# halajun/VDO_SLAM

Hardware: AMD Instinct MI355X
Metric: frames/sec (per-frame hot path, KITTI-0000-shaped 1242x375) + ms/LM-iter (batch factor graph) (higher is better)
Workload: dtype f64 (LM, RANSAC) / u8,i32,f32 (front-end, tracking)

## Files before the change

### vdo_slam_amd/csrc/orb.hip

```cpp
#include <algorithm>
#include <atomic>
#include <chrono>
#include <cmath>
#include <condition_variable>
#include <functional>
#include <memory>
#include <mutex>
#include <thread>
#include <cstring>
#include <vector>

#include "../../include/vdo_slam_hip.h"
#include "ctx.hpp"
#include "host_pool.hpp"
#include "orb_match.hpp"
#include "orb_pattern.hpp"

namespace vdo {

constexpr int kEdge = 19, kHalfPatch = 15, kPatch = 31;
constexpr int kSpecCand = 24576;
constexpr int kMaxCellDim = 68;
static_assert(kMaxCellDim <= 128, "k_fast_cells packs cell-local coordinates in 7 bits");

// ... 532 lines not shown
      int best = idx[n.b];
      float mr = resp[best];
      for (int k = n.b + 1; k < n.e; ++k) if (resp[idx[k]] > mr) { best = idx[k]; mr = resp[best]; }
      out.push_back(best);
    }
  }

 private:
  const float *x = nullptr, *y = nullptr, *resp = nullptr;
  std::vector<int> idx, tmp, ini_cnt, ini_fill;
  std::vector<int> cls;
  std::vector<QNode> nodes;
  std::vector<std::pair<int, int>> sizeAndNode, prevSN;
  int head = -1, tail = -1, count = 0;
  int push_back(const QNode& n) {
    nodes.push_back(n);
    const int id = (int)nodes.size() - 1;
    nodes[id].prev = tail; nodes[id].next = -1;
    if (tail != -1) nodes[tail].next = id; else head = id;
    tail = id; ++count;
    return id;
  }
  int push_front(const QNode& n) {
    nodes.push_back(n);
    const int id = (int)nodes.size() - 1;
    nodes[id].prev = -1; nodes[id].next = head;
    if (head != -1) nodes[head].prev = id; else tail = id;
    head = id; ++count;
    return id;
  }
  void erase(int id) {
    const QNode n = nodes[id];
    if (n.prev != -1) nodes[n.prev].next = n.next; else head = n.next;
    if (n.next != -1) nodes[n.next].prev = n.prev; else tail = n.prev;
    --count;
  }
  void divide_and_add(int id, int* nToExpand) {
    QNode c[4];
    const QNode n = nodes[id];
    const int halfX = (int)std::ceil((float)(n.URx - n.ULx) / 2), halfY = (int)std::ceil((float)(n.BRy - n.ULy) / 2);
    QNode &n1 = c[0], &n2 = c[1], &n3 = c[2], &n4 = c[3];
    n1.ULx = n.ULx; n1.ULy = n.ULy; n1.URx = n.ULx + halfX; n1.URy = n.ULy; n1.BLx = n.ULx; n1.BLy = n.ULy + halfY; n1.BRx = n.ULx + halfX; n1.BRy = n.ULy + halfY;
    n2.ULx = n1.URx; n2.ULy = n1.URy; n2.URx = n.URx; n2.URy = n.URy; n2.BLx = n1.BRx; n2.BLy = n1.BRy; n2.BRx = n.URx; n2.BRy = n.ULy + halfY;
    n3.ULx = n1.BLx; n3.ULy = n1.BLy; n3.URx = n1.BRx; n3.URy = n1.BRy; n3.BLx = n.BLx; n3.BLy = n.BLy; n3.BRx = n1.BRx; n3.BRy = n.BLy;
    n4.ULx = n3.URx; n4.ULy = n3.URy; n4.URx = n2.BRx; n4.URy = n2.BRy; n4.BLx = n3.BRx; n4.BLy = n3.BRy; n4.BRx = n.BRx; n4.BRy = n.BRy;
    int cnt[4] = {0, 0, 0, 0};
    const float sx = (float)n1.URx, sy = (float)n1.BRy;
    for (int k = n.b; k < n.e; ++k) {
      const int ki = idx[k];
      const int q = (x[ki] < sx) ? ((y[ki] < sy) ? 0 : 2) : ((y[ki] < sy) ? 1 : 3);
      cls[k] = q; ++cnt[q];
    }
    int cur[4];
    cur[0] = n.b; cur[1] = cur[0] + cnt[0]; cur[2] = cur[1] + cnt[1]; cur[3] = cur[2] + cnt[2];
    for (int q = 0; q < 4; ++q) { c[q].b = cur[q]; c[q].e = cur[q] + cnt[q]; c[q].noMore = cnt[q] == 1; }
    for (int k = n.b; k < n.e; ++k) tmp[cur[cls[k]]++] = idx[k];
    std::memcpy(idx.data() + n.b, tmp.data() + n.b, sizeof(int) * (size_t)(n.e - n.b));
    for (int q = 0; q < 4; ++q) {
      if (cnt[q] == 0) continue;
      const int nid = push_front(c[q]);
      if (cnt[q] > 1) {
        if (nToExpand) ++*nToExpand;
        sizeAndNode.push_back(std::make_pair(cnt[q], nid));
      }
    }
  }
};

constexpr int kQtThreads = 1024, kQtMaxNodes = 1024, kQtLdsKeys = 4096, kQtMaxCand = 32768, kQtMaxRounds = 48;
enum { kQtOk = 0, kQtHostLevel = 1, kQtCandOverflow = 2, kQtNodeOverflow = 3, kQtRoundCap = 4, kQtBadStrip = 5 };
struct QtDesc {
  int on_device;
  int N, nIni, H;
  int node_cap;
  int cand_cap;
  int koff;
  int out_off;
  float hX;
  float scale;
  int pad[2];
};
typedef unsigned long long qt_u64;

__device__ __forceinline__ int qt_field(qt_u64 v, int q) { return (int)((v >> (16 * q)) & 0xffffu); }
__device__ __forceinline__ int qt_nchild(qt_u64 v) { return (qt_field(v, 0) != 0) + (qt_field(v, 1) != 0) + (qt_field(v, 2) != 0) + (qt_field(v, 3) != 0); }
__device__ __forceinline__ int qt_nexp(qt_u64 v) { return (qt_field(v, 0) > 1) + (qt_field(v, 1) > 1) + (qt_field(v, 2) > 1) + (qt_field(v, 3) > 1); }

__device__ __forceinline__ qt_u64 qt_block_scan(qt_u64 v, qt_u64* s_w, qt_u64& total) {
  const int lane = threadIdx.x & 63, wv = threadIdx.x >> 6;
  qt_u64 inc = v;
#pragma unroll
  for (int off = 1; off < 64; off <<= 1) { const qt_u64 u = __shfl_up(inc, off, 64); if (lane >= off) inc += u; }
  __syncthreads();
  if (lane == 63) s_w[wv] = inc;
  __syncthreads();
  qt_u64 base = 0, tot = 0;
#pragma unroll
  for (int w = 0; w < kQtThreads / 64; ++w) { const qt_u64 p = s_w[w]; if (w < wv) base += p; tot += p; }
  total = tot;
  return base + inc - v;
}

__global__ __launch_bounds__(kQtThreads) void k_quadtree(const QtDesc* __restrict__ qd, const int* __restrict__ level_cnt,
                                                         const float* __restrict__ ox, const float* __restrict__ oy, const float* __restrict__ oresp,
                                                         uint32_t* wi, qt_u64* wp, int* __restrict__ dsel, int* __restrict__ dhdr,
                                                         int* __restrict__ hsel, int* __restrict__ hhdr) {
  __shared__ uint32_t s_nx[2][kQtMaxNodes], s_ny[2][kQtMaxNodes];
  __shared__ int s_b[2][kQtMaxNodes], s_e[2][kQtMaxNodes], s_cid[2][kQtMaxNodes];
  __shared__ qt_u64 s_qc[kQtMaxNodes];
  __shared__ qt_u64 s_sc[kQtMaxNodes];
  __shared__ int s_rank[kQtMaxNodes], s_order[kQtMaxNodes], s_nb[kQtMaxNodes];
  __shared__ qt_u64 s_w[kQtThreads / 64];
  __shared__ int s_m;
  __shared__ uint32_t s_xy[kQtLdsKeys];
  __shared__ uint16_t s_idx[2][kQtLdsKeys], s_kn[2][kQtLdsKeys];
  __shared__ qt_u64 s_P[kQtLdsKeys + 1];
  __shared__ uint8_t s_resp[kQtLdsKeys];
  const int l = blockIdx.x, t = threadIdx.x;
  const QtDesc D = qd[l];
  auto finish = [&](int status, int count) { if (t == 0) { dhdr[l] = hhdr[l] = count; dhdr[16 + l] = hhdr[16 + l] = status; } };
  if (!D.on_device) { finish(kQtHostLevel, 0); return; }
  int pos = 0;
  for (int q = 0; q < l; ++q) pos += level_cnt[q];
  const int n = level_cnt[l];
  if (n > D.cand_cap) { finish(kQtCandOverflow, 0); return; }
  if (n <= 0) { finish(kQtOk, 0); return; }
  const float *x = ox + pos, *y = oy + pos, *resp = oresp + pos;
  const int KC = (n + kQtThreads - 1) / kQtThreads;
  const int k0 = min(t * KC, n), k1 = min(k0 + KC, n);
  const int N = D.N, cap = D.node_cap;

  const bool lds_keys = n <= kQtLdsKeys;
  auto run = [&](uint32_t* xy, uint16_t* idA, uint16_t* idB, uint16_t* knA, uint16_t* knB, qt_u64* P) __attribute__((always_inline)) {
    {
      int bad = 0;
      for (int k = k0; k < k1; ++k) {
        const float fx = x[k], fy = y[k];
        const int s = (int)__fdiv_rn(fx, D.hX);
        bad |= (s < 0 || s >= D.nIni || !(fx >= 0.f && fx < 65536.f && fy >= 0.f && fy < 65536.f));
        xy[k] = (uint32_t)(int)fx | ((uint32_t)(int)fy << 16);
        if (lds_keys) { const float r = resp[k]; bad |= !(r >= 0.f && r < 256.f); s_resp[k] = (uint8_t)(int)r; }
      }
      if (__syncthreads_or(bad)) { finish(kQtBadStrip, 0); return; }
      int base = 0;
      for (int g = 0; g < D.nIni; g += 4) {
        qt_u64 a = 0;
        for (int k = k0; k < k1; ++k) { const int s = (int)__fdiv_rn((float)(xy[k] & 0xffffu), D.hX) - g; if (s >= 0 && s < 4) a += 1ull << (16 * s); }
        qt_u64 tot;
        qt_u64 ex = qt_block_scan(a, s_w, tot);
        int st[5];
        st[0] = base;
        for (int j = 0; j < 4; ++j) st[j + 1] = st[j] + qt_field(tot, j);
        for (int k = k0; k < k1; ++k) {
          const int s = (int)__fdiv_rn((float)(xy[k] & 0xffffu), D.hX) - g;
          if (s < 0 || s >= 4) continue;
          const int p = st[s] + qt_field(ex, s);
          if ((unsigned)p < (unsigned)n) { idA[p] = (uint16_t)k; knA[p] = (uint16_t)(g + s); }
          ex += 1ull << (16 * s);
        }
        if (t < 4 && g + t < D.nIni) {
          const int i = g + t;
          const int sx0 = (int)(D.hX * (float)i), sx1 = (int)(D.hX * (float)(i + 1));
          s_nx[1][i] = (uint32_t)sx0 | ((uint32_t)sx1 << 16); s_ny[1][i] = (uint32_t)D.H << 16;
          s_b[1][i] = st[t]; s_e[1][i] = st[t + 1];
        }
        base = st[4];
      }
      __syncthreads();
    }
    int count;
    {
      const int NC = (D.nIni + kQtThreads - 1) / kQtThreads;
      const int i0 = min(t * NC, D.nIni), i1 = min(i0 + NC, D.nIni);
      int a = 0;
      for (int i = i0; i < i1; ++i) a += s_e[1][i] > s_b[1][i];
      qt_u64 tot;
      int ex = (int)qt_block_scan((qt_u64)a, s_w, tot);
      count = (int)tot;
      for (int i = i0; i < i1; ++i) {
        s_nb[i] = ex;
        if (s_e[1][i] > s_b[1][i]) { s_nx[0][ex] = s_nx[1][i]; s_ny[0][ex] = s_ny[1][i]; s_b[0][ex] = s_b[1][i]; s_e[0][ex] = s_e[1][i]; s_cid[0][ex] = i; ++ex; }
      }
      __syncthreads();
      for (int k = k0; k < k1; ++k) knA[k] = (uint16_t)s_nb[knA[k]];
      __syncthreads();
    }
    int c = 0, next_cid = D.nIni;
    bool final_phase = false;
    for (int round = 0;; ++round) {
      if (round >= kQtMaxRounds) { finish(kQtRoundCap, 0); return; }
      const int o = c ^ 1;
      const uint16_t *idc = c ? idB : idA, *knc = c ? knB : knA;
      uint16_t *ido = c ? idA : idB, *kno = c ? knA : knB;
      {
        auto quadrant = [&](int k) {
          const int i = knc[k];
          if (s_e[c][i] - s_b[c][i] <= 1) return 4;
          const uint32_t nx = s_nx[c][i], ny = s_ny[c][i];
          const int x0 = (int)(nx & 0xffffu), x1 = (int)(nx >> 16), y0 = (int)(ny & 0xffffu), y1 = (int)(ny >> 16);
          const int mx = x0 + ((x1 - x0 + 1) >> 1), my = y0 + ((y1 - y0 + 1) >> 1);
          const uint32_t v = xy[idc[k]];
          const int kx = (int)(v & 0xffffu), ky = (int)(v >> 16);
          return (kx < mx) ? ((ky < my) ? 0 : 2) : ((ky < my) ? 1 : 3);
        };
        qt_u64 a = 0;
        uint32_t qs = 0;
        for (int k = k0; k < k1; ++k) { const int q = quadrant(k); if (q < 4) a += 1ull << (16 * q); if (k - k0 < 8) qs |= (uint32_t)q << (4 * (k - k0)); }
        qt_u64 tot;
        qt_u64 ex = qt_block_scan(a, s_w, tot);
        for (int k = k0; k < k1; ++k) { P[k] = ex; const int q = k - k0 < 8 ? (int)((qs >> (4 * (k - k0))) & 15u) : quadrant(k); if (q < 4) ex += 1ull << (16 * q); }
        if (t == 0) P[n] = tot;
        __syncthreads();
      }
      const int NC = (count + kQtThreads - 1) / kQtThreads;
      const int i0 = min(t * NC, count), i1 = min(i0 + NC, count);
      int E;
      {
        int a = 0;
        for (int i = i0; i < i1; ++i) {
          const int b = s_b[c][i], e = s_e[c][i];
          const bool ex = e - b > 1;
          s_qc[i] = ex ? P[e] - P[b] : 0ull;
          a += ex;
        }
        qt_u64 tot;
        int r = (int)qt_block_scan((qt_u64)a, s_w, tot);
        E = (int)tot;
        if (!final_phase) {
          for (int i = i0; i < i1; ++i) {
            if (s_e[c][i] - s_b[c][i] <= 1) { s_rank[i] = -1; continue; }
            s_rank[i] = r; s_order[r] = i; ++r;
          }
        } else {
          for (int i = i0; i < i1; ++i) {
            const int sz = s_e[c][i] - s_b[c][i];
            s_sc[i] = sz > 1 ? ((qt_u64)sz << 32) | (uint32_t)s_cid[c][i] : 0ull;
            s_rank[i] = sz > 1 ? 0 : -1;
          }
          __syncthreads();
          const int G = max(1, kQtThreads / count), per = kQtThreads / G, part = t % G;
          for (int i = t / G; i < count; i += per) {
            const qt_u64 ki = s_sc[i];
            if (!ki) continue;
            int rk = 0;
#pragma unroll 4
            for (int j = part; j < count; j += G) rk += s_sc[j] > ki;
            if (rk) atomicAdd(&s_rank[i], rk);
          }
          __syncthreads();
          for (int i = i0; i < i1; ++i) if (s_rank[i] >= 0) s_order[s_rank[i]] = i;
        }
        if (t == 0) s_m = E;
        __syncthreads();
      }
      {
        const int RC = (E + kQtThreads - 1) / kQtThreads;
        const int r0 = min(t * RC, E), r1 = min(r0 + RC, E);
        qt_u64 a = 0;
        for (int r = r0; r < r1; ++r) { const qt_u64 qc = s_qc[s_order[r]]; a += (qt_u64)qt_nchild(qc) | ((qt_u64)qt_nexp(qc) << 32); }
        qt_u64 tot;
        qt_u64 ex = qt_block_scan(a, s_w, tot);
        for (int r = r0; r < r1; ++r) {
          const qt_u64 qc = s_qc[s_order[r]];
          ex += (qt_u64)qt_nchild(qc) | ((qt_u64)qt_nexp(qc) << 32);
          s_sc[r] = ex;
          if (final_phase && count + (int)(ex & 0xffffffffu) - (r + 1) >= N) atomicMin(&s_m, r + 1);
        }
        __syncthreads();
      }
      const int m = s_m;
      const int TC = m > 0 ? (int)(s_sc[m - 1] & 0xffffffffu) : 0, n_to_expand = m > 0 ? (int)(s_sc[m - 1] >> 32) : 0;
      const int new_count = TC + count - m;
      if (new_count > cap) { finish(kQtNodeOverflow, 0); return; }
      {
        int a = 0;
        for (int i = i0; i < i1; ++i) { const int rk = s_rank[i]; a += !(rk >= 0 && rk < m); }
        qt_u64 tot;
        int u = (int)qt_block_scan((qt_u64)a, s_w, tot);
        for (int i = i0; i < i1; ++i) {
          const int rk = s_rank[i];
          if (!(rk >= 0 && rk < m)) {
            const int p = TC + u++;
            s_nx[o][p] = s_nx[c][i]; s_ny[o][p] = s_ny[c][i]; s_b[o][p] = s_b[c][i]; s_e[o][p] = s_e[c][i]; s_cid[o][p] = s_cid[c][i];
            s_nb[i] = p;
            continue;
          }
          const qt_u64 qc = s_qc[i];
          const int incl = (int)(s_sc[rk] & 0xffffffffu), nch = qt_nchild(qc);
          const int nbase = TC - incl;
          s_nb[i] = nbase;
          const uint32_t nx = s_nx[c][i], ny = s_ny[c][i];
          const int x0 = (int)(nx & 0xffffu), x1 = (int)(nx >> 16), y0 = (int)(ny & 0xffffu), y1 = (int)(ny >> 16);
          const int mx = x0 + ((x1 - x0 + 1) >> 1), my = y0 + ((y1 - y0 + 1) >> 1);
          int b = s_b[c][i], made = 0;
          for (int q = 0; q < 4; ++q) {
            const int sz = qt_field(qc, q);
            if (!sz) continue;
            const int p = nbase + nch - 1 - made;
            s_nx[o][p] = (q & 1) ? ((uint32_t)mx | ((uint32_t)x1 << 16)) : ((uint32_t)x0 | ((uint32_t)mx << 16));
            s_ny[o][p] = (q & 2) ? ((uint32_t)my | ((uint32_t)y1 << 16)) : ((uint32_t)y0 | ((uint32_t)my << 16));
            s_b[o][p] = b; s_e[o][p] = b + sz; s_cid[o][p] = next_cid + incl - nch + made;
            b += sz; ++made;
          }
        }
        __syncthreads();
      }
      for (int k = k0; k < k1; ++k) {
        const int i = knc[k], rk = s_rank[i];
        int nk = k, nn = s_nb[i];
        if (rk >= 0 && rk < m) {
          const qt_u64 qc = s_qc[i], pk = P[k], d = P[k + 1] - pk;
          const int q = (d & 0xffffu) ? 0 : ((d >> 16) & 0xffffu) ? 1 : ((d >> 32) & 0xffffu) ? 2 : 3;
          const int b = s_b[c][i];
          int offq = 0, after = 0;
          for (int j = 0; j < 4; ++j) { const int sz = qt_field(qc, j); if (j < q) offq += sz; else if (j > q) after += sz != 0; }
          nk = b + offq + qt_field(pk, q) - qt_field(P[b], q);
          nn += after;
        }
        if ((unsigned)nk < (unsigned)n) { ido[nk] = idc[k]; kno[nk] = (uint16_t)nn; }
      }
      __syncthreads();
      c = o; next_cid += TC;
      const int prev = count;
      count = new_count;
      if (count >= N || count == prev) break;
      if (!final_phase && count + 3 * n_to_expand > N) final_phase = true;
    }
    const uint16_t* idc = c ? idB : idA;
    for (int i = t; i < count; i += kQtThreads) {
      const int b = s_b[c][i], e = s_e[c][i];
      int best = idc[b];
      if (lds_keys) {
        int mr = s_resp[best];
        for (int k = b + 1; k < e; ++k) { const int ki = idc[k], r = s_resp[ki]; if (r > mr) { best = ki; mr = r; } }
      } else {
        float mr = resp[best];
        for (int k = b + 1; k < e; ++k) { const int ki = idc[k]; const float r = resp[ki]; if (r > mr) { best = ki; mr = r; } }
      }
      hsel[D.out_off + i] = best; dsel[D.out_off + i] = pos + best;
    }
    finish(kQtOk, count);
  };
  if (n <= kQtLdsKeys) run(s_xy, s_idx[0], s_idx[1], s_kn[0], s_kn[1], s_P);
  else {
    uint32_t* const w0 = wi + 3 * (size_t)D.koff;
    uint16_t* const h0 = (uint16_t*)(w0 + D.cand_cap);
    run(w0, h0, h0 + D.cand_cap, h0 + 2 * (size_t)D.cand_cap, h0 + 3 * (size_t)D.cand_cap, wp + D.koff + l);
  }
}

__global__ __launch_bounds__(256) void k_qt_rows(const QtDesc* __restrict__ qd, int n_levels, const int* __restrict__ dhdr, const int* __restrict__ dsel,
                                                 const float* __restrict__ ox, const float* __restrict__ oy, const float* __restrict__ oresp,
                                                 const uint8_t* __restrict__ pyr, const LevelDesc* __restrict__ levels, UMax um, float* __restrict__ hrows, int row_pitch) {
  const int lane = threadIdx.x & 31;
  const int slot = (blockIdx.x * 256 + threadIdx.x) >> 5;
  int l = -1;
  for (int q = 0; q < n_levels; ++q) { const int off = qd[q].out_off; if (qd[q].on_device && slot >= off && slot < off + qd[q].node_cap) l = q; }
  const bool valid = l >= 0 && dhdr[16 + l] == kQtOk && slot - qd[l].out_off < dhdr[l];
  int m10 = 0, m01 = 0, kx = 0, ky = 0, dense = 0;
  if (valid) {
    dense = dsel[slot];
    kx = (int)ox[dense]; ky = (int)oy[dense];
    if (lane < 31) {
      const LevelDesc L = levels[l];
      const int v = lane - kHalfPatch;
      const int d = um.v[v < 0 ? -v : v];
      const uint8_t* row = pyr + L.off_inner + (size_t)(ky + (kEdge - 3) + v) * L.bw + (kx + (kEdge - 3));
      int px[kPatch];
#pragma unroll
      for (int u = 0; u < kPatch; ++u) px[u] = row[u - kHalfPatch];
      int rs = 0;
#pragma unroll
      for (int u = 0; u < kPatch; ++u) { const int uu = u - kHalfPatch; const int p = (uu >= -d && uu <= d) ? px[u] : 0; m10 += uu * p; rs += p; }
      m01 = v * rs;
    }
  }
#pragma unroll
  for (int off = 16; off > 0; off >>= 1) { m10 += __shfl_down(m10, off, 32); m01 += __shfl_down(m01, off, 32); }
  if (valid && lane == 0) {
    const float ang = fast_atan2_dev((float)m01, (float)m10);
    float fx = (float)kx + (float)(kEdge - 3), fy = (float)ky + (float)(kEdge - 3);
    if (l != 0) { const float sc = qd[l].scale; fx = fx * sc; fy = fy * sc; }
    float* r = hrows + slot;
    r[0] = fx; r[row_pitch] = fy; r[2 * (size_t)row_pitch] = oresp[dense]; r[3 * (size_t)row_pitch] = ang;
  }
}

}

using namespace vdo;

struct vdo_orb {
  vdo_ctx* ctx = nullptr;
  vdo_orb_params prm{};
  int w = 0, h = 0, ncells = 0;
  int max_kp = 0;
  int cell_cap = 1;
  std::vector<LevelDesc> levels;
  std::vector<CellDesc> cells;
  std::vector<int> cell_level, nfeat;
  std::vector<float> scale;
  UMax um{};
  Blur7 blur{};
  PyrDesc pyr{};
  PyrDesc pyr2{};
  std::vector<void*> allocs;
  uint8_t *d_src = nullptr, *d_pyr = nullptr, *d_blur = nullptr;
  LevelDesc* d_levels = nullptr; CellDesc* d_cells = nullptr; int* d_cell_level = nullptr;
  int *d_cnt = nullptr, *d_offs = nullptr, *d_level_cnt = nullptr; uint32_t* d_pack = nullptr;
  float *d_x = nullptr, *d_y = nullptr, *d_resp = nullptr, *d_ang = nullptr; int* d_lvl = nullptr;
  int64_t pyr_bytes = 0, blur_bytes = 0;
  int dense_cap = 0;
  std::vector<int> sel_dense;
  OrbPattern* d_pat = nullptr; int* d_sel = nullptr; uint8_t* d_desc = nullptr; int desc_cap = 0;
  bool desc_ready = false, pos_ready = false;
  float *m_x = nullptr, *m_y = nullptr; int32_t* m_oct = nullptr; int match_cap = 0;
  float* h_pin = nullptr; float* d_pin = nullptr;
  bool fused_angle = false;
  const float *hx = nullptr, *hy = nullptr, *hresp = nullptr, *hang = nullptr; std::vector<int> hlevel_cnt;
  int n_cand = 0;
  QuadTree qt[16];
  std::vector<int> sel[16];
  std::unique_ptr<LevelPool> pool;
  bool dev_tree = false;
  bool ang_queued = false;
  QtDesc qtd[16]; QtDesc* d_qtd = nullptr;
  int qt_out = 0;
  uint32_t* d_qt_i = nullptr; int *d_qsel = nullptr, *d_qhdr = nullptr; qt_u64* d_qt_p = nullptr;
  double ms_device = 0, ms_tree = 0;
  bool begun = false;
// ... 618 lines not shown
  if (n_features) *n_features = o->nfeat[level];
  if (n_candidates) *n_candidates = o->hlevel_cnt.empty() ? 0 : o->hlevel_cnt[level];
  return VDO_OK;
}

extern "C" int vdo_orb_get_pyramid(vdo_orb* o, int level, uint8_t* out_bordered) {
  if (!o || !out_bordered || level < 0 || level >= o->prm.n_levels) return set_error(VDO_ERR_INVALID, "bad argument");
  int rc = ctx_bind(o->ctx);
  if (rc != VDO_OK) return rc;
  const LevelDesc& L = o->levels[level];
  if (hipMemcpy(out_bordered, o->d_pyr + L.off, (size_t)L.bw * L.bh, hipMemcpyDeviceToHost) != hipSuccess) return set_error(VDO_ERR_NO_DEVICE, "D2H failed");
  return VDO_OK;
}

extern "C" int vdo_orb_get_blurred(vdo_orb* o, int level, uint8_t* out) {
  if (!o || !out || level < 0 || level >= o->prm.n_levels) return set_error(VDO_ERR_INVALID, "bad argument");
  int rc = ctx_bind(o->ctx);
  if (rc != VDO_OK) return rc;
  int64_t boff = 0;
  for (int l = 0; l < level; ++l) boff += (int64_t)o->levels[l].w * o->levels[l].h;
  const LevelDesc& L = o->levels[level];
  hipStreamSynchronize(o->ctx->stream);
  if (hipMemcpy(out, o->d_blur + boff, (size_t)L.w * L.h, hipMemcpyDeviceToHost) != hipSuccess) return set_error(VDO_ERR_NO_DEVICE, "D2H failed");
  return VDO_OK;
}

extern "C" int vdo_orb_get_candidates(vdo_orb* o, int level, float* x, float* y, float* resp, float* angle, int cap, int* n) {
  if (!o || !n || level < 0 || level >= o->prm.n_levels || o->hlevel_cnt.empty()) return set_error(VDO_ERR_INVALID, "bad argument / no extraction yet");
  int pos = 0;
  for (int l = 0; l < level; ++l) pos += o->hlevel_cnt[l];
  const int cnt = o->hlevel_cnt[level];
  *n = cnt;
  if (angle && !o->fused_angle && !o->begun) {
    const int rc = ctx_bind(o->ctx);
    if (rc != VDO_OK) return rc;
    orb_ensure_angles(o);
  }
  if (angle && !o->fused_angle && !o->begun && hipEventSynchronize(o->ev_ang) != hipSuccess) return set_error(VDO_ERR_NO_DEVICE, "orb angle stage failed: %s", hipGetErrorString(hipGetLastError()));
  for (int k = 0; k < cnt && k < cap; ++k) {
    if (x) x[k] = o->hx[pos + k];
    if (y) y[k] = o->hy[pos + k];
    if (resp) resp[k] = o->hresp[pos + k];
    if (angle) angle[k] = o->hang[pos + k];
  }
  return VDO_OK;
}

extern "C" int vdo_depth_preprocess(vdo_ctx* ctx, float* depth, int64_t n, float bf, float factor, int is_device) {
  if (!ctx || !depth || n <= 0) return set_error(VDO_ERR_INVALID, "bad argument");
  int rc = ctx_bind(ctx);
  if (rc != VDO_OK) return rc;
  hipStream_t s = ctx->stream;
  float* d = depth;
  if (!is_device) {
    if (hipMalloc((void**)&d, 4 * (size_t)n) != hipSuccess) return set_error(VDO_ERR_OOM, "hipMalloc failed");
    hipMemcpyAsync(d, depth, 4 * (size_t)n, hipMemcpyHostToDevice, s);
  }
  hipLaunchKernelGGL(k_depth_preprocess, dim3((unsigned)((n + 255) / 256)), dim3(256), 0, s, d, n, bf, factor);
  if (!is_device) {
    hipMemcpyAsync(depth, d, 4 * (size_t)n, hipMemcpyDeviceToHost, s);
    hipStreamSynchronize(s);
    hipFree(d);
  }
  hipError_t e = hipGetLastError();
  if (e != hipSuccess) return set_error(VDO_ERR_NO_DEVICE, "depth preprocess: %s", hipGetErrorString(e));
  return VDO_OK;
}

extern "C" int vdo_rgb2gray(vdo_ctx* ctx, const uint8_t* rgb, int64_t n_pixels, int channels, int rgb_order, uint8_t* gray) {
  if (!ctx || !rgb || !gray || n_pixels <= 0 || (channels != 3 && channels != 4)) return set_error(VDO_ERR_INVALID, "bad argument");
  int rc = ctx_bind(ctx);
  if (rc != VDO_OK) return rc;
  hipStream_t s = ctx->stream;
  uint8_t *ds = nullptr, *dd = nullptr;
  if (hipMalloc((void**)&ds, (size_t)n_pixels * channels) != hipSuccess || hipMalloc((void**)&dd, (size_t)n_pixels) != hipSuccess) { if (ds) hipFree(ds); return set_error(VDO_ERR_OOM, "hipMalloc failed"); }
  hipMemcpyAsync(ds, rgb, (size_t)n_pixels * channels, hipMemcpyHostToDevice, s);
  hipLaunchKernelGGL(k_rgb2gray, dim3((unsigned)((n_pixels + 255) / 256)), dim3(256), 0, s, (const uint8_t*)ds, n_pixels, channels, rgb_order, dd);
  hipMemcpyAsync(gray, dd, (size_t)n_pixels, hipMemcpyDeviceToHost, s);
  hipError_t e = hipStreamSynchronize(s);
  hipFree(ds); hipFree(dd);
  if (e != hipSuccess) return set_error(VDO_ERR_NO_DEVICE, "rgb2gray: %s", hipGetErrorString(e));
  return VDO_OK;
}
```

Measured before the change: 1497.

## Restructure quadtree kernel with DPP block scans and one-node-per-thread rounds

Replaces the shuffle-based block prefix scan with DPP row/wave scans and readlane, which removes one barrier per scan and double-buffers the wave-total slots. The per-round node processing now maps one node per thread, fusing the separate count/rank/child scans into a single packed scan. Keys and node ids, and node begin/end, are packed into 32-bit words, and the split points are cached. Candidate loops are batched by four to overlap LDS loads. It also adds an optional compile-time profiling hook. The DPP control codes and the packing assumptions add correctness risk.

```diff
diff --git a/vdo_slam_amd/csrc/orb.hip b/vdo_slam_amd/csrc/orb.hip
--- a/vdo_slam_amd/csrc/orb.hip
+++ b/vdo_slam_amd/csrc/orb.hip
@@ -638,23 +638,59 @@
 };
 typedef unsigned long long qt_u64;
 
-__device__ __forceinline__ int qt_field(qt_u64 v, int q) { return (int)((v >> (16 * q)) & 0xffffu); }
+#ifdef QT_PROFILE
+constexpr int kQtProfCap = 1024;
+__device__ long long g_qt_prof[4 + 2 * kQtProfCap];
+#define QT_STAMP(id)                                                                                      \
+  do {                                                                                                    \
+    if (blockIdx.x == 0 && threadIdx.x == 0 && qt_pn < kQtProfCap) {                                      \
+      if (qt_pn == 0) g_qt_prof[1] = (long long)wall_clock64();                                           \
+      g_qt_prof[4 + 2 * qt_pn] = (id); g_qt_prof[5 + 2 * qt_pn] = (long long)clock64();                   \
+      g_qt_prof[0] = ++qt_pn; g_qt_prof[2] = (long long)wall_clock64();                                   \
+    }                                                                                                     \
+  } while (0)
+#else
+#define QT_STAMP(id) do {} while (0)
+#endif
+
+__device__ __forceinline__ int qt_field(qt_u64 v, int q) { const uint32_t h = (q & 2) ? (uint32_t)(v >> 32) : (uint32_t)v; return (int)((h >> ((q & 1) << 4)) & 0xffffu); }
 __device__ __forceinline__ int qt_nchild(qt_u64 v) { return (qt_field(v, 0) != 0) + (qt_field(v, 1) != 0) + (qt_field(v, 2) != 0) + (qt_field(v, 3) != 0); }
 __device__ __forceinline__ int qt_nexp(qt_u64 v) { return (qt_field(v, 0) > 1) + (qt_field(v, 1) > 1) + (qt_field(v, 2) > 1) + (qt_field(v, 3) > 1); }
 
+static_assert(kQtMaxCand < 65536 && 4 * kQtMaxNodes < 65536, "a field of a packed scan word overflows into its neighbour: the halves can no longer be scanned apart");
+static_assert(kQtThreads / 64 == 16 && kQtMaxNodes <= kQtThreads, "16 wave totals = one DPP row; one node per thread");
+template <int CTRL, int ROWS>
+__device__ __forceinline__ uint32_t qt_dpp(uint32_t v) { return (uint32_t)__builtin_amdgcn_update_dpp(0, (int)v, CTRL, ROWS, 0xF, false); }
+__device__ __forceinline__ uint32_t qt_row_scan(uint32_t v) {
+  v += qt_dpp<0x111, 0xF>(v); v += qt_dpp<0x112, 0xF>(v); v += qt_dpp<0x114, 0xF>(v); v += qt_dpp<0x118, 0xF>(v);
+  return v;
+}
+__device__ __forceinline__ uint32_t qt_wave_scan(uint32_t v) {
+  v = qt_row_scan(v);
+  v += qt_dpp<0x142, 0xA>(v); v += qt_dpp<0x143, 0xC>(v);
+  return v;
+}
 __device__ __forceinline__ qt_u64 qt_block_scan(qt_u64 v, qt_u64* s_w, qt_u64& total) {
-  const int lane = threadIdx.x & 63, wv = threadIdx.x >> 6;
-  qt_u64 inc = v;
-#pragma unroll
-  for (int off = 1; off < 64; off <<= 1) { const qt_u64 u = __shfl_up(inc, off, 64); if (lane >= off) inc += u; }
-  __syncthreads();
+  const int lane = threadIdx.x & 63, wv = __builtin_amdgcn_readfirstlane((int)(threadIdx.x >> 6));
+  const qt_u64 inc = (qt_u64)qt_wave_scan((uint32_t)v) | ((qt_u64)qt_wave_scan((uint32_t)(v >> 32)) << 32);
   if (lane == 63) s_w[wv] = inc;
   __syncthreads();
-  qt_u64 base = 0, tot = 0;
-#pragma unroll
-  for (int w = 0; w < kQtThreads / 64; ++w) { const qt_u64 p = s_w[w]; if (w < wv) base += p; tot += p; }
-  total = tot;
-  return base + inc - v;
+  const qt_u64 p = s_w[lane & 15];
+  const uint32_t lo = qt_row_scan((uint32_t)p), hi = qt_row_scan((uint32_t)(p >> 32));
+  total = (qt_u64)(uint32_t)__builtin_amdgcn_readlane((int)lo, 15) | ((qt_u64)(uint32_t)__builtin_amdgcn_readlane((int)hi, 15) << 32);
+  const int pw = wv > 0 ? wv - 1 : 0;
+  const qt_u64 before = (qt_u64)(uint32_t)__builtin_amdgcn_readlane((int)lo, pw) | ((qt_u64)(uint32_t)__builtin_amdgcn_readlane((int)hi, pw) << 32);
+  return (wv > 0 ? before : 0ull) + inc - v;
+}
+__device__ __forceinline__ int qt_block_scan32(int v, qt_u64* s_w, int& total) {
+  const int lane = threadIdx.x & 63, wv = __builtin_amdgcn_readfirstlane((int)(threadIdx.x >> 6));
+  const uint32_t inc = qt_wave_scan((uint32_t)v);
+  if (lane == 63) s_w[wv] = inc;
+  __syncthreads();
+  const uint32_t lo = qt_row_scan((uint32_t)s_w[lane & 15]);
+  total = __builtin_amdgcn_readlane((int)lo, 15);
+  const int before = __builtin_amdgcn_readlane((int)lo, wv > 0 ? wv - 1 : 0);
+  return (wv > 0 ? before : 0) + (int)inc - v;
 }
 
 __global__ __launch_bounds__(kQtThreads) void k_quadtree(const QtDesc* __restrict__ qd, const int* __restrict__ level_cnt,
@@ -662,246 +698,296 @@
                                                          uint32_t* wi, qt_u64* wp, int* __restrict__ dsel, int* __restrict__ dhdr,
                                                          int* __restrict__ hsel, int* __restrict__ hhdr) {
   __shared__ uint32_t s_nx[2][kQtMaxNodes], s_ny[2][kQtMaxNodes];
-  __shared__ int s_b[2][kQtMaxNodes], s_e[2][kQtMaxNodes], s_cid[2][kQtMaxNodes];
-  __shared__ qt_u64 s_qc[kQtMaxNodes];
-  __shared__ qt_u64 s_sc[kQtMaxNodes];
-  __shared__ int s_rank[kQtMaxNodes], s_order[kQtMaxNodes], s_nb[kQtMaxNodes];
-  __shared__ qt_u64 s_w[kQtThreads / 64];
+  __shared__ uint32_t s_be[2][kQtMaxNodes];
+  __shared__ uint32_t s_sp[2][kQtMaxNodes];
+  __shared__ int s_cid[2][kQtMaxNodes];
+  __shared__ qt_u64 s_qo[kQtMaxNodes], s_nn[kQtMaxNodes];
+  __shared__ uint16_t s_cn[kQtMaxNodes];
+  __shared__ alignas(16) qt_u64 s_sc[kQtMaxNodes];
+  __shared__ int s_rank[kQtMaxNodes], s_order[kQtMaxNodes];
+  __shared__ qt_u64 s_w[2][kQtThreads / 64];
   __shared__ int s_m;
   __shared__ uint32_t s_xy[kQtLdsKeys];
-  __shared__ uint16_t s_idx[2][kQtLdsKeys], s_kn[2][kQtLdsKeys];
+  __shared__ uint32_t s_ik[2][kQtLdsKeys];
   __shared__ qt_u64 s_P[kQtLdsKeys + 1];
   __shared__ uint8_t s_resp[kQtLdsKeys];
   const int l = blockIdx.x, t = threadIdx.x;
+#ifdef QT_PROFILE
+  int qt_pn = 0;
+#endif
+  QT_STAMP(0);
   const QtDesc D = qd[l];
-  auto finish = [&](int status, int count) { if (t == 0) { dhdr[l] = hhdr[l] = count; dhdr[16 + l] = hhdr[16 + l] = status; } };
-  if (!D.on_device) { finish(kQtHostLevel, 0); return; }
   int pos = 0;
   for (int q = 0; q < l; ++q) pos += level_cnt[q];
   const int n = level_cnt[l];
+  auto finish = [&](int status, int count) { if (t == 0) { dhdr[l] = hhdr[l] = count; dhdr[16 + l] = hhdr[16 + l] = status; } };
+  if (!D.on_device) { finish(kQtHostLevel, 0); return; }
   if (n > D.cand_cap) { finish(kQtCandOverflow, 0); return; }
   if (n <= 0) { finish(kQtOk, 0); return; }
   const float *x = ox + pos, *y = oy + pos, *resp = oresp + pos;
   const int KC = (n + kQtThreads - 1) / kQtThreads;
   const int k0 = min(t * KC, n), k1 = min(k0 + KC, n);
   const int N = D.N, cap = D.node_cap;
+  int sw = 0;
+  auto split = [](uint32_t nx, uint32_t ny) {
+    const uint32_t x0 = nx & 0xffffu, x1 = nx >> 16, y0 = ny & 0xffffu, y1 = ny >> 16;
+    return (x0 + ((x1 - x0 + 1) >> 1)) | ((y0 + ((y1 - y0 + 1) >> 1)) << 16);
+  };
 
   const bool lds_keys = n <= kQtLdsKeys;
-  auto run = [&](uint32_t* xy, uint16_t* idA, uint16_t* idB, uint16_t* knA, uint16_t* knB, qt_u64* P) __attribute__((always_inline)) {
+  auto run = [&](uint32_t* xy, uint32_t* ikA, uint32_t* ikB, qt_u64* P) __attribute__((always_inline)) {
     {
       int bad = 0;
-      for (int k = k0; k < k1; ++k) {
-        const float fx = x[k], fy = y[k];
-        const int s = (int)__fdiv_rn(fx, D.hX);
-        bad |= (s < 0 || s >= D.nIni || !(fx >= 0.f && fx < 65536.f && fy >= 0.f && fy < 65536.f));
-        xy[k] = (uint32_t)(int)fx | ((uint32_t)(int)fy << 16);
-        if (lds_keys) { const float r = resp[k]; bad |= !(r >= 0.f && r < 256.f); s_resp[k] = (uint8_t)(int)r; }
+      for (int kb = t; kb < n; kb += 4 * kQtThreads) {
+        float fx[4], fy[4], fr[4];
+#pragma unroll
+        for (int j = 0; j < 4; ++j) { const int k = min(kb + j * kQtThreads, n - 1); fx[j] = x[k]; fy[j] = y[k]; fr[j] = resp[k]; }
+#pragma unroll
+        for (int j = 0; j < 4; ++j) {
+          const int k = kb + j * kQtThreads;
+          if (k >= n) continue;
+          const int s = (int)__fdiv_rn(fx[j], D.hX);
+          bad |= (s < 0 || s >= D.nIni || !(fx[j] >= 0.f && fx[j] < 65536.f && fy[j] >= 0.f && fy[j] < 65536.f));
+          xy[k] = (uint32_t)(int)fx[j] | ((uint32_t)(int)fy[j] << 16);
+          if (lds_keys) { bad |= !(fr[j] >= 0.f && fr[j] < 256.f); s_resp[k] = (uint8_t)(int)fr[j]; }
+        }
       }
       if (__syncthreads_or(bad)) { finish(kQtBadStrip, 0); return; }
+    }
+    QT_STAMP(1);
+    {
       int base = 0;
       for (int g = 0; g < D.nIni; g += 4) {
         qt_u64 a = 0;
-        for (int k = k0; k < k1; ++k) { const int s = (int)__fdiv_rn((float)(xy[k] & 0xffffu), D.hX) - g; if (s >= 0 && s < 4) a += 1ull << (16 * s); }
+        uint32_t ss = 0;
+        for (int k = k0; k < k1; ++k) {
+          int s = (int)__fdiv_rn((float)(xy[k] & 0xffffu), D.hX) - g;
+          if (s < 0 || s >= 4) s = 4; else a += 1ull << (16 * s);
+          if (k - k0 < 8) ss |= (uint32_t)s << (4 * (k - k0));
+        }
         qt_u64 tot;
-        qt_u64 ex = qt_block_scan(a, s_w, tot);
+        qt_u64 ex = qt_block_scan(a, s_w[sw ^= 1], tot);
         int st[5];
         st[0] = base;
         for (int j = 0; j < 4; ++j) st[j + 1] = st[j] + qt_field(tot, j);
         for (int k = k0; k < k1; ++k) {
-          const int s = (int)__fdiv_rn((float)(xy[k] & 0xffffu), D.hX) - g;
+          const int s = k - k0 < 8 ? (int)((ss >> (4 * (k - k0))) & 15u) : (int)__fdiv_rn((float)(xy[k] & 0xffffu), D.hX) - g;
           if (s < 0 || s >= 4) continue;
           const int p = st[s] + qt_field(ex, s);
-          if ((unsigned)p < (unsigned)n) { idA[p] = (uint16_t)k; knA[p] = (uint16_t)(g + s); }
+          if ((unsigned)p < (unsigned)n) ikA[p] = (uint32_t)k | ((uint32_t)(g + s) << 16);
           ex += 1ull << (16 * s);
         }
         if (t < 4 && g + t < D.nIni) {
           const int i = g + t;
           const int sx0 = (int)(D.hX * (float)i), sx1 = (int)(D.hX * (float)(i + 1));
           s_nx[1][i] = (uint32_t)sx0 | ((uint32_t)sx1 << 16); s_ny[1][i] = (uint32_t)D.H << 16;
-          s_b[1][i] = st[t]; s_e[1][i] = st[t + 1];
+          s_be[1][i] = (uint32_t)st[t] | ((uint32_t)st[t + 1] << 16);
         }
         base = st[4];
       }
       __syncthreads();
     }
+    QT_STAMP(2);
     int count;
     {
-      const int NC = (D.nIni + kQtThreads - 1) / kQtThreads;
-      const int i0 = min(t * NC, D.nIni), i1 = min(i0 + NC, D.nIni);
-      int a = 0;
-      for (int i = i0; i < i1; ++i) a += s_e[1][i] > s_b[1][i];
-      qt_u64 tot;
-      int ex = (int)qt_block_scan((qt_u64)a, s_w, tot);
-      count = (int)tot;
-      for (int i = i0; i < i1; ++i) {
-        s_nb[i] = ex;
-        if (s_e[1][i] > s_b[1][i]) { s_nx[0][ex] = s_nx[1][i]; s_ny[0][ex] = s_ny[1][i]; s_b[0][ex] = s_b[1][i]; s_e[0][ex] = s_e[1][i]; s_cid[0][ex] = i; ++ex; }
+      const uint32_t be = t < D.nIni ? s_be[1][t] : 0u;
+      const int ne = (be >> 16) > (be & 0xffffu);
+      const int ex = qt_block_scan32(ne, s_w[sw ^= 1], count);
+      if (t < D.nIni) {
+        s_rank[t] = ex | ((int)(be >> 16) - (int)(be & 0xffffu) > 1 ? 0x8000 : 0);
+        if (ne) { const uint32_t nx = s_nx[1][t], ny = s_ny[1][t]; s_nx[0][ex] = nx; s_ny[0][ex] = ny; s_be[0][ex] = be; s_sp[0][ex] = split(nx, ny); s_cid[0][ex] = t; }
       }
       __syncthreads();
-      for (int k = k0; k < k1; ++k) knA[k] = (uint16_t)s_nb[knA[k]];
+      for (int k = k0; k < k1; ++k) { const uint32_t w = ikA[k]; ikA[k] = (w & 0xffffu) | ((uint32_t)s_rank[w >> 16] << 16); }
       __syncthreads();
     }
+    QT_STAMP(3);
     int c = 0, next_cid = D.nIni;
     bool final_phase = false;
     for (int round = 0;; ++round) {
       if (round >= kQtMaxRounds) { finish(kQtRoundCap, 0); return; }
       const int o = c ^ 1;
-      const uint16_t *idc = c ? idB : idA, *knc = c ? knB : knA;
-      uint16_t *ido = c ? idA : idB, *kno = c ? knA : knB;
+      const uint32_t* ikc = c ? ikB : ikA;
+      uint32_t* iko = c ? ikA : ikB;
+      auto quadrants = [&](int kb, int (&q)[4]) {
+        uint32_t w[4], sp[4], v[4];
+#pragma unroll
+        for (int j = 0; j < 4; ++j) w[j] = ikc[min(kb + j, n - 1)];
+#pragma unroll
+        for (int j = 0; j < 4; ++j) { sp[j] = s_sp[c][(w[j] >> 16) & 0x7fffu]; v[j] = xy[min((int)(w[j] & 0xffffu), n - 1)]; }
+#pragma unroll
+        for (int j = 0; j < 4; ++j) {
+          const bool divides = (w[j] >> 31) && kb + j < k1;
+          const int qq = ((v[j] & 0xffffu) < (sp[j] & 0xffffu)) ? (((v[j] >> 16) < (sp[j] >> 16)) ? 0 : 2) : (((v[j] >> 16) < (sp[j] >> 16)) ? 1 : 3);
+          q[j] = divides ? qq : 4;
+        }
+      };
+      uint32_t qs = 0;
       {
-        auto quadrant = [&](int k) {
-          const int i = knc[k];
-          if (s_e[c][i] - s_b[c][i] <= 1) return 4;
-          const uint32_t nx = s_nx[c][i], ny = s_ny[c][i];
-          const int x0 = (int)(nx & 0xffffu), x1 = (int)(nx >> 16), y0 = (int)(ny & 0xffffu), y1 = (int)(ny >> 16);
-          const int mx = x0 + ((x1 - x0 + 1) >> 1), my = y0 + ((y1 - y0 + 1) >> 1);
-          const uint32_t v = xy[idc[k]];
-          const int kx = (int)(v & 0xffffu), ky = (int)(v >> 16);
-          return (kx < mx) ? ((ky < my) ? 0 : 2) : ((ky < my) ? 1 : 3);
-        };
         qt_u64 a = 0;
-        uint32_t qs = 0;
-        for (int k = k0; k < k1; ++k) { const int q = quadrant(k); if (q < 4) a += 1ull << (16 * q); if (k - k0 < 8) qs |= (uint32_t)q << (4 * (k - k0)); }
+        for (int kb = k0; kb < k1; kb += 4) {
+          int q[4];
+          quadrants(kb, q);
+#pragma unroll
+          for (int j = 0; j < 4; ++j) { if (q[j] < 4) a += 1ull << (16 * q[j]); if (kb - k0 < 8) qs |= (uint32_t)q[j] << (4 * (kb - k0 + j)); }
+        }
         qt_u64 tot;
-        qt_u64 ex = qt_block_scan(a, s_w, tot);
-        for (int k = k0; k < k1; ++k) { P[k] = ex; const int q = k - k0 < 8 ? (int)((qs >> (4 * (k - k0))) & 15u) : quadrant(k); if (q < 4) ex += 1ull << (16 * q); }
+        qt_u64 ex = qt_block_scan(a, s_w[sw ^= 1], tot);
+        for (int kb = k0; kb < k1; kb += 4) {
+          int q[4];
+          if (kb - k0 < 8) {
+#pragma unroll
+            for (int j = 0; j < 4; ++j) q[j] = (int)((qs >> (4 * (kb - k0 + j))) & 15u);
+          } else quadrants(kb, q);
+#pragma unroll
+          for (int j = 0; j < 4; ++j) if (kb + j < k1) { P[kb + j] = ex; if (q[j] < 4) ex += 1ull << (16 * q[j]); }
+        }
         if (t == 0) P[n] = tot;
         __syncthreads();
       }
-      const int NC = (count + kQtThreads - 1) / kQtThreads;
-      const int i0 = min(t * NC, count), i1 = min(i0 + NC, count);
-      int E;
-      {
-        int a = 0;
-        for (int i = i0; i < i1; ++i) {
-          const int b = s_b[c][i], e = s_e[c][i];
-          const bool ex = e - b > 1;
-          s_qc[i] = ex ? P[e] - P[b] : 0ull;
-          a += ex;
+      QT_STAMP(10);
+      const bool in_list = t < count;
+      const uint32_t be = in_list ? s_be[c][t] : 0u;
+      const int nb = (int)(be & 0xffffu);
+      const bool expandable = (int)(be >> 16) - nb > 1;
+      const qt_u64 Pb = expandable ? P[nb] : 0ull;
+      const qt_u64 qc = expandable ? P[be >> 16] - Pb : 0ull;
+      const int nch = qt_nchild(qc), nxp = qt_nexp(qc);
+      int m, TC, n_to_expand, incl, u;
+      bool processed;
+      if (!final_phase) {
+        qt_u64 tot;
+        const qt_u64 pre = qt_block_scan((qt_u64)expandable | ((qt_u64)nch << 16) | ((qt_u64)nxp << 32), s_w[sw ^= 1], tot);
+        m = (int)(tot & 0xffffu); TC = (int)((tot >> 16) & 0xffffu); n_to_expand = (int)(tot >> 32);
+        processed = expandable;
+        incl = (int)((pre >> 16) & 0xffffu) + nch;
+        u = t - (int)(pre & 0xffffu);
+        QT_STAMP(11);
+      } else {
+        static_assert(kQtMaxNodes * (kQtMaxRounds + 1) <= 65536 && kQtMaxCand < 65536, "size << 16 | creation id no longer fits the 32-bit rank key");
+        uint32_t* const s_key = (uint32_t*)s_sc;
+        s_key[t] = expandable ? ((uint32_t)((int)(be >> 16) - nb) << 16) | (uint32_t)s_cid[c][t] : 0u;
+        if (in_list) { s_cn[t] = (uint16_t)(nch | (nxp << 8)); s_rank[t] = expandable ? 0 : -1; }
+        const int E = __syncthreads_count(expandable);
+        const int G = max(1, kQtThreads / count), per = kQtThreads / G, part = t % G;
+        const int quads = (count + 3) >> 2;
+        const uint4* k4 = (const uint4*)s_sc;
+        for (int i = t / G; i < count; i += per) {
+          const uint32_t ki = s_key[i];
+          if (!ki) continue;
+          int rk = 0;
+#pragma unroll 1
+          for (int j = part; j < quads; j += G) { const uint4 v = k4[j]; rk += (int)(v.x > ki) + (int)(v.y > ki) + (int)(v.z > ki) + (int)(v.w > ki); }
+          if (rk) atomicAdd(&s_rank[i], rk);
         }
-        qt_u64 tot;
-        int r = (int)qt_block_scan((qt_u64)a, s_w, tot);
-        E = (int)tot;
-        if (!final_phase) {
-          for (int i = i0; i < i1; ++i) {
-            if (s_e[c][i] - s_b[c][i] <= 1) { s_rank[i] = -1; continue; }
-            s_rank[i] = r; s_order[r] = i; ++r;
-          }
-        } else {
-          for (int i = i0; i < i1; ++i) {
-            const int sz = s_e[c][i] - s_b[c][i];
-            s_sc[i] = sz > 1 ? ((qt_u64)sz << 32) | (uint32_t)s_cid[c][i] : 0ull;
-            s_rank[i] = sz > 1 ? 0 : -1;
+        __syncthreads();
+        const int rk = in_list ? s_rank[t] : -1;
+        if (rk >= 0) s_order[rk] = t;
+        if (t == 0) s_m = E;
+        __syncthreads();
+        QT_STAMP(15);
+        {
+          const uint32_t cn = t < E ? s_cn[s_order[t]] : 0u;
+          const qt_u64 a = (qt_u64)(cn & 0xffu) | ((qt_u64)(cn >> 8) << 32);
+          qt_u64 tot;
+          const qt_u64 inc = qt_block_scan(a, s_w[sw ^= 1], tot) + a;
+          if (t < E) {
+            s_sc[t] = inc;
+            if (count + (int)(inc & 0xffffffffu) - (t + 1) >= N) atomicMin(&s_m, t + 1);
           }
           __syncthreads();
-          const int G = max(1, kQtThreads / count), per = kQtThreads / G, part = t % G;
-          for (int i = t / G; i < count; i += per) {
-            const qt_u64 ki = s_sc[i];
-            if (!ki) continue;
-            int rk = 0;
-#pragma unroll 4
-            for (int j = part; j < count; j += G) rk += s_sc[j] > ki;
-            if (rk) atomicAdd(&s_rank[i], rk);
-          }
-          __syncthreads();
-          for (int i = i0; i < i1; ++i) if (s_rank[i] >= 0) s_order[s_rank[i]] = i;
         }
-        if (t == 0) s_m = E;
-        __syncthreads();
+        m = s_m;
+        TC = m > 0 ? (int)(s_sc[m - 1] & 0xffffffffu) : 0; n_to_expand = m > 0 ? (int)(s_sc[m - 1] >> 32) : 0;
+        processed = rk >= 0 && rk < m;
+        incl = processed ? (int)(s_sc[rk] & 0xffffffffu) : 0;
+        QT_STAMP(12);
+        int tot;
+        u = qt_block_scan32(in_list && !processed, s_w[sw ^= 1], tot);
       }
-      {
-        const int RC = (E + kQtThreads - 1) / kQtThreads;
-        const int r0 = min(t * RC, E), r1 = min(r0 + RC, E);
-        qt_u64 a = 0;
-        for (int r = r0; r < r1; ++r) { const qt_u64 qc = s_qc[s_order[r]]; a += (qt_u64)qt_nchild(qc) | ((qt_u64)qt_nexp(qc) << 32); }
-        qt_u64 tot;
-        qt_u64 ex = qt_block_scan(a, s_w, tot);
-        for (int r = r0; r < r1; ++r) {
-          const qt_u64 qc = s_qc[s_order[r]];
-          ex += (qt_u64)qt_nchild(qc) | ((qt_u64)qt_nexp(qc) << 32);
-          s_sc[r] = ex;
-          if (final_phase && count + (int)(ex & 0xffffffffu) - (r + 1) >= N) atomicMin(&s_m, r + 1);
-        }
-        __syncthreads();
-      }
-      const int m = s_m;
-      const int TC = m > 0 ? (int)(s_sc[m - 1] & 0xffffffffu) : 0, n_to_expand = m > 0 ? (int)(s_sc[m - 1] >> 32) : 0;
       const int new_count = TC + count - m;
       if (new_count > cap) { finish(kQtNodeOverflow, 0); return; }
-      {
-        int a = 0;
-        for (int i = i0; i < i1; ++i) { const int rk = s_rank[i]; a += !(rk >= 0 && rk < m); }
-        qt_u64 tot;
-        int u = (int)qt_block_scan((qt_u64)a, s_w, tot);
-        for (int i = i0; i < i1; ++i) {
-          const int rk = s_rank[i];
-          if (!(rk >= 0 && rk < m)) {
-            const int p = TC + u++;
-            s_nx[o][p] = s_nx[c][i]; s_ny[o][p] = s_ny[c][i]; s_b[o][p] = s_b[c][i]; s_e[o][p] = s_e[c][i]; s_cid[o][p] = s_cid[c][i];
-            s_nb[i] = p;
-            continue;
-          }
-          const qt_u64 qc = s_qc[i];
-          const int incl = (int)(s_sc[rk] & 0xffffffffu), nch = qt_nchild(qc);
+      if (in_list) {
+        if (!processed) {
+          const int p = TC + u;
+          s_nx[o][p] = s_nx[c][t]; s_ny[o][p] = s_ny[c][t]; s_be[o][p] = be; s_sp[o][p] = s_sp[c][t]; s_cid[o][p] = s_cid[c][t];
+          s_nn[t] = (qt_u64)((uint32_t)p | (expandable ? 0x8000u : 0u));
+          s_qo[t] = ~0ull;
+        } else {
           const int nbase = TC - incl;
-          s_nb[i] = nbase;
-          const uint32_t nx = s_nx[c][i], ny = s_ny[c][i];
-          const int x0 = (int)(nx & 0xffffu), x1 = (int)(nx >> 16), y0 = (int)(ny & 0xffffu), y1 = (int)(ny >> 16);
-          const int mx = x0 + ((x1 - x0 + 1) >> 1), my = y0 + ((y1 - y0 + 1) >> 1);
-          int b = s_b[c][i], made = 0;
+          const uint32_t nx = s_nx[c][t], ny = s_ny[c][t], sp = s_sp[c][t];
+          const uint32_t x0 = nx & 0xffffu, x1 = nx >> 16, y0 = ny & 0xffffu, y1 = ny >> 16, mx = sp & 0xffffu, my = sp >> 16;
+          int b = nb, made = 0;
+          qt_u64 qo = 0, nnw = 0;
+#pragma unroll
           for (int q = 0; q < 4; ++q) {
             const int sz = qt_field(qc, q);
             if (!sz) continue;
             const int p = nbase + nch - 1 - made;
-            s_nx[o][p] = (q & 1) ? ((uint32_t)mx | ((uint32_t)x1 << 16)) : ((uint32_t)x0 | ((uint32_t)mx << 16));
-            s_ny[o][p] = (q & 2) ? ((uint32_t)my | ((uint32_t)y1 << 16)) : ((uint32_t)y0 | ((uint32_t)my << 16));
-            s_b[o][p] = b; s_e[o][p] = b + sz; s_cid[o][p] = next_cid + incl - nch + made;
+            qo |= (qt_u64)(uint32_t)(b - qt_field(Pb, q)) << (16 * q);
+            nnw |= (qt_u64)((uint32_t)p | (sz > 1 ? 0x8000u : 0u)) << (16 * q);
+            const uint32_t cx = (q & 1) ? (mx | (x1 << 16)) : (x0 | (mx << 16)), cy = (q & 2) ? (my | (y1 << 16)) : (y0 | (my << 16));
+            s_nx[o][p] = cx; s_ny[o][p] = cy; s_sp[o][p] = split(cx, cy);
+            s_be[o][p] = (uint32_t)b | ((uint32_t)(b + sz) << 16); s_cid[o][p] = next_cid + incl - nch + made;
             b += sz; ++made;
           }
+          s_qo[t] = qo; s_nn[t] = nnw;
         }
-        __syncthreads();
-      }
-      for (int k = k0; k < k1; ++k) {
-        const int i = knc[k], rk = s_rank[i];
-        int nk = k, nn = s_nb[i];
-        if (rk >= 0 && rk < m) {
-          const qt_u64 qc = s_qc[i], pk = P[k], d = P[k + 1] - pk;
-          const int q = (d & 0xffffu) ? 0 : ((d >> 16) & 0xffffu) ? 1 : ((d >> 32) & 0xffffu) ? 2 : 3;
-          const int b = s_b[c][i];
-          int offq = 0, after = 0;
-          for (int j = 0; j < 4; ++j) { const int sz = qt_field(qc, j); if (j < q) offq += sz; else if (j > q) after += sz != 0; }
-          nk = b + offq + qt_field(pk, q) - qt_field(P[b], q);
-          nn += after;
-        }
-        if ((unsigned)nk < (unsigned)n) { ido[nk] = idc[k]; kno[nk] = (uint16_t)nn; }
       }
       __syncthreads();
+      QT_STAMP(13);
+      for (int kb = k0; kb < k1; kb += 4) {
+        uint32_t w[4];
+        qt_u64 pk[4], qo[4], nnw[4];
+#pragma unroll
+        for (int j = 0; j < 4; ++j) { const int k = min(kb + j, n - 1); w[j] = ikc[k]; pk[j] = P[k]; }
+#pragma unroll
+        for (int j = 0; j < 4; ++j) { const int i = (int)((w[j] >> 16) & 0x7fffu); qo[j] = s_qo[i]; nnw[j] = s_nn[i]; }
+#pragma unroll
+        for (int j = 0; j < 4; ++j) {
+          const int k = kb + j;
+          if (k >= k1) continue;
+          int nk = k;
+          uint32_t nn = (uint32_t)nnw[j] & 0xffffu;
+          if (qo[j] != ~0ull) {
+            int q;
+            if (kb - k0 < 8) q = (int)((qs >> (4 * (kb - k0 + j))) & 15u);
+            else { const qt_u64 d = P[k + 1] - pk[j]; q = (d & 0xffffu) ? 0 : ((d >> 16) & 0xffffu) ? 1 : ((d >> 32) & 0xffffu) ? 2 : 3; }
+            nk = qt_field(qo[j], q) + qt_field(pk[j], q);
+            nn = (uint32_t)qt_field(nnw[j], q);
+          }
+          if ((unsigned)nk < (unsigned)n) iko[nk] = (w[j] & 0xffffu) | (nn << 16);
+        }
+      }
+      __syncthreads();
+      QT_STAMP(14);
       c = o; next_cid += TC;
       const int prev = count;
       count = new_count;
       if (count >= N || count == prev) break;
       if (!final_phase && count + 3 * n_to_expand > N) final_phase = true;
     }
-    const uint16_t* idc = c ? idB : idA;
-    for (int i = t; i < count; i += kQtThreads) {
-      const int b = s_b[c][i], e = s_e[c][i];
-      int best = idc[b];
+    if (t < count) {
+      const uint32_t* ikc = c ? ikB : ikA;
+      const uint32_t be = s_be[c][t];
+      const int b = (int)(be & 0xffffu), e = (int)(be >> 16);
+      int best = (int)(ikc[b] & 0xffffu);
       if (lds_keys) {
         int mr = s_resp[best];
-        for (int k = b + 1; k < e; ++k) { const int ki = idc[k], r = s_resp[ki]; if (r > mr) { best = ki; mr = r; } }
+        for (int k = b + 1; k < e; ++k) { const int ki = (int)(ikc[k] & 0xffffu), r = s_resp[ki]; if (r > mr) { best = ki; mr = r; } }
       } else {
         float mr = resp[best];
-        for (int k = b + 1; k < e; ++k) { const int ki = idc[k]; const float r = resp[ki]; if (r > mr) { best = ki; mr = r; } }
+        for (int k = b + 1; k < e; ++k) { const int ki = (int)(ikc[k] & 0xffffu); const float r = resp[ki]; if (r > mr) { best = ki; mr = r; } }
       }
-      hsel[D.out_off + i] = best; dsel[D.out_off + i] = pos + best;
-    }
+      hsel[D.out_off + t] = best; dsel[D.out_off + t] = pos + best;
+    }
+    QT_STAMP(20);
     finish(kQtOk, count);
   };
-  if (n <= kQtLdsKeys) run(s_xy, s_idx[0], s_idx[1], s_kn[0], s_kn[1], s_P);
+  if (n <= kQtLdsKeys) run(s_xy, s_ik[0], s_ik[1], s_P);
   else {
     uint32_t* const w0 = wi + 3 * (size_t)D.koff;
-    uint16_t* const h0 = (uint16_t*)(w0 + D.cand_cap);
-    run(w0, h0, h0 + D.cand_cap, h0 + 2 * (size_t)D.cand_cap, h0 + 3 * (size_t)D.cand_cap, wp + D.koff + l);
+    run(w0, w0 + D.cand_cap, w0 + 2 * (size_t)D.cand_cap, wp + D.koff + l);
   }
 }
 
@@ -1686,3 +1772,13 @@
   if (e != hipSuccess) return set_error(VDO_ERR_NO_DEVICE, "rgb2gray: %s", hipGetErrorString(e));
   return VDO_OK;
 }
+
+#ifdef QT_PROFILE
+extern "C" int vdo_orb_qt_profile(long long* out, int cap) {
+  if (!out || cap <= 0) return set_error(VDO_ERR_INVALID, "vdo_orb_qt_profile: no buffer");
+  const size_t nb = sizeof(long long) * (size_t)std::min(cap, 4 + 2 * vdo::kQtProfCap);
+  if (hipDeviceSynchronize() != hipSuccess || hipMemcpyFromSymbol(out, HIP_SYMBOL(vdo::g_qt_prof), nb) != hipSuccess)
+    return set_error(VDO_ERR_NO_DEVICE, "vdo_orb_qt_profile: copy failed");
+  return VDO_OK;
+}
+#endif
```

Result: slower. 1459 (-2.5%).
